# ZHANGKEON/DIS-YOLO

Hardware: AMD Instinct MI355X
Metric: train images/sec @576x576 bf16 (higher is better)
Workload: dtype bf16

## Files before the change

dis-yolo_amd/csrc/conv_common.h:

```cpp
#pragma once
#include <utility>
#include "common.h"

namespace dyconv {
struct ConvParams {
  const bf16* x0;
  const bf16* x1;
  const bf16* w;
  const float* scale;
  const float* shift;
  const bf16* residual;
  void* y;
  float* stats;
  const bf16* bn_x;
  const float* bn_scale;
  const float* bn_shift;
  const float* bn_mean;
  const float* bn_rstd;
  float* bn_part;
  float bn_alpha;
  int B, H, W, C0, C1, Cin;
  int Ho, Wo, Cout;
  int ks, stride, pad_t, pad_l, dmask, dshift;
  int M, K, nk;
// ... 7 lines not shown
  float alpha;
  void* y_act;
  const float* gamma;
  const float* beta;
  float* mm;
  float* mv;
  float* o_scale;
  float* o_shift;
  float* o_mean;
  float* o_rstd;
  float* dgamma;
  float* dbeta;
  unsigned* csync;
  float bn_decay, bn_eps;
  double inv_count;
};

template <int BK>
static __device__ __forceinline__ int swz(int row, int chunk) {
  if (BK == 32) return chunk ^ ((0x78 >> (((row >> 2) & 3) * 2)) & 3);
  return chunk ^ ((row >> 1) & 7);
}

static __device__ __forceinline__ int swz_any(int row, int chunk) { return chunk ^ (((row >> 2) & 1) << 1); }

typedef int i32x4 __attribute__((ext_vector_type(4)));
constexpr unsigned OOB = 0x80000000u;
template <int LDS_IMM>
static __device__ __forceinline__ void dma16(unsigned voff, i32x4 srd, unsigned soff, unsigned lds_base) {
  asm volatile("s_mov_b32 m0, %3\n\ts_nop 0\n\tbuffer_load_dwordx4 %0, %1, %2 offen lds"
// ... 183 lines not shown
```

dis-yolo_amd/csrc/conv_igemm.hip:

```cpp
#include <utility>
#include "common.h"
#include "conv_common.h"
#include "runtime.h"

using namespace dyconv;

namespace {

template <int BM, int BN, int WM, int WN, int BK, int ST, int KS, int KG = 1, int EPI = 0>
__global__ __launch_bounds__(WM* WN * 64 * KG, (BM == 128 && BN == 128) ? 3 : 1) void conv_igemm_kernel(ConvParams p) {
#ifdef HALO_PROBE
  long long gp_t[5];
  gp_t[0] = (long long)__builtin_amdgcn_s_memtime();
  gp_t[4] = (long long)__builtin_amdgcn_s_memrealtime();
#endif
  constexpr int NW = WM * WN;
  constexpr int T = NW * 64;
  constexpr int WTM = BM / WM, WTN = BN / WN;
  constexpr int MI = WTM / 16, NI = WTN / 16;
  constexpr int ROWB = BK * 2;
  constexpr int CPR = ROWB / 16;
  constexpr int SLAB = 1024 * NW;
  constexpr int A_BYTES = (BM * ROWB + SLAB - 1) / SLAB * SLAB;
  constexpr int B_BYTES = (BN * ROWB + SLAB - 1) / SLAB * SLAB;
// ... 1439 lines not shown
        const int idx = r_ * 64 + lane;
        const int r16 = idx / CPR8, ch = idx % CPR8;
        const int m = __shfl(m_of[t], r16, 64);
        const int n = n0 + ch * 8;
        const uint4 o = *reinterpret_cast<const uint4*>(sw + (t * 16 + r16) * ROWP + ch * 16);
        unsigned off = (m >= 0 && n < p.Cout) ? (unsigned)(((size_t)m * p.Cout + n) * 2) : OOB;
#ifdef DY_PROBE
        if (p.flags & 0x80000) off = OOB;
#endif
        buffer_store16(o, off, srdy);
      }
    }
  }
}

template <int NI>
__global__ __launch_bounds__(512) void conv1x1_stream_kernel(ConvParams p, int ngroups) {
  constexpr int NW = 8, U = 2;
  constexpr int BN = NI * 16;
  constexpr int ROWP = BN * 2 + 16;
  constexpr int STG = U * 16 * ROWP;
  constexpr int MAXKS = 6;
  extern __shared__ __attribute__((aligned(16))) char smem[];
  const int tid = threadIdx.x;
  const int lane = tid & 63;
  const int wave = __builtin_amdgcn_readfirstlane(tid >> 6);
  const int frow = lane & 15, cq = lane >> 4;
  const int K = p.K, ks32 = K >> 5;
  const int wpitch = K * 2 + 16;
  char* const wl = smem;
  char* const stg = smem + ((BN * wpitch + 15) & ~15);
  for (int c = tid; c < BN * (K >> 3); c += NW * 64) {
    const int n = c / (K >> 3), kc = c - n * (K >> 3);
    uint4 v = uint4{0, 0, 0, 0};
    if (n < p.Cout) v = *reinterpret_cast<const uint4*>(p.w + (size_t)n * K + kc * 8);
    *reinterpret_cast<uint4*>(wl + n * wpitch + kc * 16) = v;
  }
  float esc[NI][4], esh[NI][4];
#pragma unroll
  for (int j = 0; j < NI; ++j)
#pragma unroll
    for (int r = 0; r < 4; ++r) {
      const int n = j * 16 + cq * 4 + r;
      esc[j][r] = (p.scale && n < p.Cout) ? p.scale[n] : 1.f;
      esh[j][r] = (p.shift && n < p.Cout) ? p.shift[n] : 0.f;
    }
  __syncthreads();
  const bool f32out = p.flags & DISYOLO_CONV_OUT_F32;
  const bool do_stats = p.flags & DISYOLO_CONV_STATS;
  const bool vec_ok = (p.Cout & 7) == 0;
  const bool use_res = p.residual != nullptr;
  const int H1 = p.H >> 1, W1 = p.W >> 1;
  const int ks0 = p.C0 >> 5;
  float s1[NI][4], s2[NI][4];
#pragma unroll
  for (int j = 0; j < NI; ++j)
#pragma unroll
    for (int r = 0; r < 4; ++r) s1[j][r] = s2[j][r] = 0.f;
  char* const sw = stg + wave * STG;

  for (int g = blockIdx.x * NW + wave; g < ngroups; g += gridDim.x * NW) {
    int m_of[U];
    bf16x8 xf[U][MAXKS];
#pragma unroll
// ... 10 lines not shown
        a1 = p.x1 + ((size_t)(b * H1 + (y >> 1)) * W1 + (x >> 1)) * p.C1 + cq * 8;
      }
#pragma unroll
      for (int k = 0; k < MAXKS; ++k)
        if (k < ks32) xf[u][k] = *reinterpret_cast<const bf16x8*>(k < ks0 ? a0 + k * 32 : a1 + (k - ks0) * 32);
    }
    uint2 rres[U][NI];
    if (use_res) {
#pragma unroll
      for (int u = 0; u < U; ++u)
#pragma unroll
        for (int j = 0; j < NI; ++j) {
          const int n = j * 16 + cq * 4;
          rres[u][j] = *reinterpret_cast<const uint2*>(p.residual + (size_t)(m_of[u] >= 0 ? m_of[u] : 0) * p.Cout + (n + 3 < p.Cout ? n : 0));
        }
    }
    f32x4 acc[U][NI];
#pragma unroll
    for (int u = 0; u < U; ++u)
#pragma unroll
      for (int j = 0; j < NI; ++j) acc[u][j] = f32x4{0.f, 0.f, 0.f, 0.f};
#pragma unroll
    for (int k = 0; k < MAXKS; ++k) {
      if (k < ks32) {
        bf16x8 wf[NI];
#pragma unroll
        for (int j = 0; j < NI; ++j) wf[j] = *reinterpret_cast<const bf16x8*>(wl + (j * 16 + frow) * wpitch + (k * 4 + cq) * 16);
#pragma unroll
        for (int u = 0; u < U; ++u)
#pragma unroll
// ... 37 lines not shown
            for (int r = 0; r < 4; ++r)
              if (n + r < p.Cout) {
                float o = v[r];
                if (use_res && !(n + 3 < p.Cout)) o += (float)p.residual[off + r];
                if (f32out)
                  reinterpret_cast<float*>(p.y)[off + r] = o;
                else
                  reinterpret_cast<bf16*>(p.y)[off + r] = (bf16)o;
              }
          }
        } else {
          uint2 o2;
          o2.x = pack2(v[0], v[1]);
          o2.y = pack2(v[2], v[3]);
          *reinterpret_cast<uint2*>(sw + (u * 16 + frow) * ROWP + n * 2) = o2;
        }
      }
    if (!(f32out || !vec_ok)) {
      __builtin_amdgcn_fence(__ATOMIC_RELEASE, "wavefront");
      __builtin_amdgcn_wave_barrier();
      __builtin_amdgcn_fence(__ATOMIC_ACQUIRE, "wavefront");
      constexpr int CPR8 = BN / 8;
      constexpr int RPF = (U * 16 * CPR8 + 63) / 64;
      const int cpr = p.Cout >> 3;
      bf16* yo = reinterpret_cast<bf16*>(p.y);
#pragma unroll
      for (int r_ = 0; r_ < RPF; ++r_) {
        const int idx = r_ * 64 + lane;
        const int row = idx / CPR8, ch = idx % CPR8;
        const int m = g * (U * 16) + row;
        if (idx < U * 16 * CPR8 && ch < cpr && m < p.M)
          *reinterpret_cast<uint4*>(yo + (size_t)m * p.Cout + ch * 8) = *reinterpret_cast<const uint4*>(sw + row * ROWP + ch * 16);
      }
      __builtin_amdgcn_fence(__ATOMIC_RELEASE, "wavefront");
      __builtin_amdgcn_wave_barrier();
      __builtin_amdgcn_fence(__ATOMIC_ACQUIRE, "wavefront");
    }
  }
  if (do_stats) {
    float* red = reinterpret_cast<float*>(stg + NW * STG);
#pragma unroll
    for (int j = 0; j < NI; ++j)
#pragma unroll
      for (int r = 0; r < 4; ++r) {
        float a = s1[j][r], b2 = s2[j][r];
#pragma unroll
        for (int o = 1; o < 16; o <<= 1) {
          a += __shfl_xor(a, o, 64);
          b2 += __shfl_xor(b2, o, 64);
        }
        if (frow == 0) {
          const int nl = j * 16 + cq * 4 + r;
          red[(wave * BN + nl) * 2 + 0] = a;
          red[(wave * BN + nl) * 2 + 1] = b2;
        }
      }
    __syncthreads();
    for (int nl = tid; nl < BN; nl += NW * 64) {
      if (nl < p.Cout) {
        float a = 0.f, b2 = 0.f;
#pragma unroll
        for (int w_ = 0; w_ < NW; ++w_) {
          a += red[(w_ * BN + nl) * 2 + 0];
          b2 += red[(w_ * BN + nl) * 2 + 1];
        }
        stats_out(p, blockIdx.x, nl, a, b2);
      }
    }
  }
}

struct Patch {
  int ph, pw;
};
Patch pick_patch(int H, int W, int max_frags, int max_halo) {
  Patch best{0, 0};
  int best_area = 0, best_halo = 1 << 30;
  for (int ph = 1; ph <= H; ++ph) {
    if (H % ph) continue;
    for (int pw = 1; pw <= W; ++pw) {
      if (W % pw) continue;
// ... 53 lines not shown
    if (hipGetDevice(&dev) == hipSuccess) (void)hipDeviceGetAttribute(&n, hipDeviceAttributeMultiprocessorCount, dev);
    return n > 0 ? n : 256;
  }();
  int G = ncu / q.tilesN;
  if (G < 1) G = 1;
  if (G > q.tilesM) G = q.tilesM;
  hipLaunchKernelGGL((conv_stream_kernel<NW, FW, NI>), dim3(G * q.tilesN), dim3(NW * 64), lds, s, q, pt.ph, pt.pw, tilesY,
                     tilesX, G);
  DY_CHECK_LAUNCH();
  return DISYOLO_OK;
}

bool stream1x1_ok(const disyolo_conv_desc* d) {
  if (d->ksize != 1 || d->stride != 1 || d->in_div != 1 || d->Ho != d->H || d->Wo != d->W) return false;
  if (d->Cout > 64 || d->C0 % 32 || d->C1 % 32 || d->C0 + d->C1 > 192) return false;
  if (d->flags & DISYOLO_CONV_BN_BWD_STATS) return false;
  return true;
}
int stream1x1_blocks(int M) {
  const int groups = ceil_div(M, 32);
  int blocks = ceil_div(groups, 8 * 4);
  if (blocks > 512) blocks = 512;
  if (blocks < 1) blocks = 1;
  return blocks;
}
template <int NI>
int launch_stream1x1_n(const ConvParams& p, hipStream_t s) {
  constexpr int BN = NI * 16;
  const size_t wbytes = ((size_t)BN * (p.K * 2 + 16) + 15) & ~(size_t)15;
  const size_t lds = wbytes + (size_t)8 * 2 * 16 * (BN * 2 + 16) + (size_t)8 * BN * 8;
  static bool attr_set = false;
  if (!attr_set) {
    (void)hipFuncSetAttribute(reinterpret_cast<const void*>(&conv1x1_stream_kernel<NI>), hipFuncAttributeMaxDynamicSharedMemorySize,
                              (int)(64 * (192 * 2 + 16) + 8 * 2 * 16 * (64 * 2 + 16) + 8 * 64 * 8));
    attr_set = true;
  }
  hipLaunchKernelGGL((conv1x1_stream_kernel<NI>), dim3(stream1x1_blocks(p.M)), dim3(512), lds, s, p, ceil_div(p.M, 32));
  DY_CHECK_LAUNCH();
  return DISYOLO_OK;
}
int launch_stream1x1(const ConvParams& p, hipStream_t s) {
  if (p.Cout <= 16) return launch_stream1x1_n<1>(p, s);
  if (p.Cout <= 32) return launch_stream1x1_n<2>(p, s);
  return launch_stream1x1_n<4>(p, s);
}

struct LaunchQuery {
  bool active = false, have = false, want_bwd = false, want_fused = false;
  int grid = 0, rows = 0, bn = 0, resident = 0;
};
thread_local LaunchQuery tl_query;
template <class K>
int resident_blocks(K kernel, int threads, size_t lds) {
  int dev = 0, cus = 0, occ = 0;
  if (hipGetDevice(&dev) != hipSuccess) return 0;
  if (hipDeviceGetAttribute(&cus, hipDeviceAttributeMultiprocessorCount, dev) != hipSuccess) return 0;
  if (hipOccupancyMaxActiveBlocksPerMultiprocessor(&occ, reinterpret_cast<const void*>(kernel), threads, lds) != hipSuccess) {
    (void)hipGetLastError();
    return 0;
// ... 248 lines not shown
      if (halo_ok(d, id, pt)) return sel;
    } else {
      return sel;
    }
    sel = pick_auto(d, M);
  }
  return sel;
}

extern "C" int disyolo_conv2d_bn_bwd_stats_ok(const disyolo_conv_desc* d) {
  if (!d || (d->flags & DISYOLO_CONV_OUT_F32) || d->Cout % 8) return 0;
  if (conv_c16_shape(d)) return 0;
  const int sel = resolve_sel(d, d->B * d->Ho * d->Wo, nullptr);
  int id = sel & 0xff;
  if ((id >= 16 && id < 20) || id == 24 || id == 25) return 1;
  if (!is_gemm_tile(id) || d->in_div != 1) return 0;
  {
    const char* e = getenv("DISYOLO_BN_BWD_STATS_GEMM");
    if (!(e && e[0] == '1')) return 0;
  }
  const bool bk64 = (d->C0 % 64 == 0) && (d->C1 % 64 == 0) && !(sel & 0x100);
  id = resolve_tile(id, bk64, d->ksize * d->ksize * (d->C0 + d->C1));
  if (id == 12) return 1;
  return d->ksize == 1 && (id == 1 || id == 2 || id == 3 || id == 6 || id == 9 || id == 10 || id == 11) ? 1 : 0;
}

extern "C" int disyolo_conv2d_stats_rows(const disyolo_conv_desc* d) {
  if (!d) return DISYOLO_E_ARG;
  const int M = d->B * d->Ho * d->Wo;
  if (conv_c16_shape(d)) return conv_c16_stats_rows(d);
  Patch pt;
  const int id = resolve_sel(d, M, &pt) & 0xff;
  if (id == 24 || id == 25) {
    FlatGeom g;
    return flat_ok(d, id, &g) ? g.tilesM : DISYOLO_E_ARG;
  }
  if (id == 21) return stream1x1_blocks(M);
  if (!is_gemm_tile(id)) return d->B * (d->H / pt.ph) * (d->W / pt.pw);
  const int bm = tile_bm(id);
// ... 94 lines not shown

extern "C" int disyolo_dgrad_s2_quad_ok(int B, int Hdy, int Wdy, int Cdy, int C) {
  return (B > 0 && Hdy > 0 && Wdy > 0 && Cdy % 64 == 0 && C % 8 == 0 && (4 * C) % 128 == 0 && C <= 64 &&
          (int64_t)B * Hdy * Wdy * 4 * C * 2 < (1LL << 31) && (int64_t)B * Hdy * Wdy * Cdy * 2 < (1LL << 31)) ? 1 : 0;
}

extern "C" int disyolo_dgrad_s2_quad(const void* dy, const void* wq, void* dx, const void* residual, int B, int Hdy, int Wdy,
                                     int Cdy, int C, void* stream) {
  DY_REQUIRE(dy && wq && dx, "dgrad_s2_quad: null pointer");
  DY_REQUIRE(disyolo_dgrad_s2_quad_ok(B, Hdy, Wdy, Cdy, C) == 1, "dgrad_s2_quad: needs Cdy %% 64 == 0, C in {32, 64}");
  DY_RECORD_OR_RUN([=](void* s) { return disyolo_dgrad_s2_quad(dy, wq, dx, residual, B, Hdy, Wdy, Cdy, C, s); });
  ConvParams p;
  p.x0 = (const bf16*)dy; p.x1 = nullptr; p.w = (const bf16*)wq;
  p.scale = nullptr; p.shift = nullptr; p.residual = (const bf16*)residual; p.y = dx; p.stats = nullptr;
  p.bn_x = nullptr; p.bn_scale = p.bn_shift = p.bn_mean = p.bn_rstd = nullptr; p.bn_part = nullptr; p.bn_alpha = 0.f;
  p.B = B; p.H = Hdy; p.W = Wdy; p.C0 = Cdy; p.C1 = 0; p.Cin = Cdy;
  p.Ho = Hdy; p.Wo = Wdy; p.Cout = 4 * C;
  p.ks = 3; p.stride = 1; p.pad_t = 1; p.pad_l = 1; p.dmask = 0; p.dshift = 0;
  p.M = B * Hdy * Wdy;
  p.K = 9 * Cdy;
  p.bytes0 = (unsigned)((size_t)B * Hdy * Wdy * Cdy * 2);
  p.bytes1 = 0;
  p.bytesw = (unsigned)((size_t)4 * C * 9 * Cdy * 2);
  p.nk = 0;
  p.flags = 0;
  p.alpha = 0.f;
  p.tilesM = p.tilesN = 0;
  p.xcd_n = 0; p.halo_split = 0;
  p.pcls = 0; p.Mc = 0; p.tilesMc = 0;
  p.tapmask = 0x1b;
// ... 71 lines not shown
  p.residual = (const bf16*)d->residual;
  p.y = d->y;
  p.stats = d->stats;
  p.bn_x = nullptr; p.bn_scale = p.bn_shift = p.bn_mean = p.bn_rstd = nullptr; p.bn_part = nullptr; p.bn_alpha = 0.f;
  if (d->flags & DISYOLO_CONV_BN_BWD_STATS) {
    DY_REQUIRE(d->bn_x && d->bn_scale && d->bn_shift && d->bn_mean && d->bn_rstd && d->bn_partials,
               "conv: BN_BWD_STATS flag with a null bn_* pointer");
    DY_REQUIRE((d->flags & DISYOLO_CONV_BN_BWD_FUSED) || disyolo_conv2d_bn_bwd_stats_ok(d) == 1,
               "conv: BN_BWD_STATS needs a patch kernel (tile 16-19, 24, 25 on a shape it covers) or a GEMM tile with that epilogue "
               "(ask disyolo_conv2d_bn_bwd_stats_ok), bf16 output, Cout %% 8 == 0");
    DY_REQUIRE(!(d->flags & DISYOLO_CONV_BN_BWD_FUSED) || (!(d->flags & (DISYOLO_CONV_OUT_F32 | DISYOLO_CONV_STATS | DISYOLO_CONV_LEAKY)) &&
                                                          !d->scale && !d->shift && d->Cout % 8 == 0),
               "conv: BN_BWD_FUSED needs a plain bf16 data-gradient conv (no scale / shift / LEAKY / STATS), Cout %% 8 == 0");
    p.bn_x = (const bf16*)d->bn_x; p.bn_scale = d->bn_scale; p.bn_shift = d->bn_shift; p.bn_mean = d->bn_mean;
    p.bn_rstd = d->bn_rstd; p.bn_part = d->bn_partials; p.bn_alpha = d->bn_alpha;
  }
  p.B = d->B; p.H = d->H; p.W = d->W; p.C0 = d->C0; p.C1 = d->C1; p.Cin = d->C0 + d->C1;
  p.Ho = d->Ho; p.Wo = d->Wo; p.Cout = d->Cout;
  p.ks = d->ksize; p.stride = d->stride; p.pad_t = d->pad_t; p.pad_l = d->pad_l;
  p.dmask = d->in_div - 1; p.dshift = d->in_div == 2 ? 1 : 0;
  p.M = d->B * d->Ho * d->Wo;
  p.K = d->ksize * d->ksize * p.Cin;
  p.bytes0 = (unsigned)((size_t)d->B * d->H * d->W * d->C0 * 2);
  p.bytes1 = (unsigned)((size_t)d->B * (d->H / 2) * (d->W / 2) * d->C1 * 2);
  p.bytesw = (unsigned)((size_t)d->Cout * p.K * 2);
  p.nk = 0;
  p.flags = d->flags;
  p.alpha = d->alpha;
  p.tilesM = p.tilesN = 0;
  p.xcd_n = 0; p.halo_split = 0;
// ... 34 lines not shown
```

dis-yolo_amd/lib.py:

```python
from __future__ import annotations

import ctypes as C
import os
from typing import Optional

import numpy as np
import torch

_HERE = os.path.dirname(os.path.abspath(__file__))
LIB_PATH = os.environ.get("DISYOLO_LIB", os.path.join(_HERE, "libdisyolo_hip.so"))

GRAD_LD = 32
ROI_MAX = 16
ROI_W = 12
K_MAPS = (3, 5, 7)
MASK_STRIDES = (1, 2, 4)


def roi_w(k: int) -> int:
    return 2 * (k + 1) + 4


def block32_post(k: int) -> int:
    return {3: 1, 5: 2, 7: 3}[k]
CONV_LEAKY, CONV_OUT_F32, CONV_STATS, CONV_BN_BWD_STATS, CONV_BN_FUSED, CONV_BN_BWD_FUSED = 1, 2, 4, 8, 16, 32


class DisyoloError(RuntimeError):
    pass


class ConvDesc(C.Structure):
    _fields_ = [
        ("B", C.c_int32), ("H", C.c_int32), ("W", C.c_int32),
        ("C0", C.c_int32), ("C1", C.c_int32),
        ("Ho", C.c_int32), ("Wo", C.c_int32), ("Cout", C.c_int32),
        ("ksize", C.c_int32), ("stride", C.c_int32),
        ("pad_t", C.c_int32), ("pad_l", C.c_int32),
        ("in_div", C.c_int32), ("flags", C.c_int32),
        ("alpha", C.c_float), ("tile", C.c_int32),
# ... 7 lines not shown
        ("bn_moving_mean", C.c_void_p), ("bn_moving_var", C.c_void_p),
        ("bn_out_scale", C.c_void_p), ("bn_out_shift", C.c_void_p), ("bn_out_mean", C.c_void_p), ("bn_out_rstd", C.c_void_p),
        ("bn_dgamma", C.c_void_p), ("bn_dbeta", C.c_void_p), ("cluster_sync", C.c_void_p),
    ]


_SIGS = {
    "disyolo_version": (C.c_int, []),
    "disyolo_last_error": (C.c_char_p, []),
    "disyolo_conv_desc_size": (C.c_size_t, []),
    "disyolo_find_contours": (C.c_int, [C.c_void_p, C.c_int, C.c_int, C.c_void_p, C.c_int64, C.c_void_p, C.c_void_p, C.c_int,
                                        C.POINTER(C.c_int), C.POINTER(C.c_int64)]),
    "disyolo_conv2d_stats_rows": (C.c_int, [C.POINTER(ConvDesc)]),
    "disyolo_conv2d_bn_bwd_stats_ok": (C.c_int, [C.POINTER(ConvDesc)]),
    "disyolo_conv2d_bn_fused_ok": (C.c_int, [C.POINTER(ConvDesc)]),
    "disyolo_cluster_sync_words": (C.c_int, [C.c_int]),
    "disyolo_cluster_sync_error": (C.c_int, [C.c_void_p, C.c_int]),
    "disyolo_conv2d_fwd": (C.c_int, [C.POINTER(ConvDesc), C.c_void_p]),
    "disyolo_conv2d_tile": (C.c_int, [C.POINTER(ConvDesc)] + [C.POINTER(C.c_int)] * 4),
    "disyolo_conv_first_fwd": (C.c_int, [C.c_void_p] * 5 + [C.c_int] * 4 + [C.c_float, C.c_void_p]),
    "disyolo_conv12_fused_ok": (C.c_int, [C.c_int] * 3),
    "disyolo_conv12_fused_fwd": (C.c_int, [C.c_void_p] * 8 + [C.c_int] * 3 + [C.c_float, C.c_void_p]),
    "disyolo_block32_fused_ok": (C.c_int, [C.c_int] * 6),
    "disyolo_block64_fused_ok": (C.c_int, [C.c_int] * 4),
    "disyolo_pack_quad": (C.c_int, [C.c_void_p, C.c_void_p, C.c_int, C.c_int, C.c_void_p]),
    "disyolo_dgrad_s2_quad_ok": (C.c_int, [C.c_int] * 5),
    "disyolo_dgrad_s2_quad": (C.c_int, [C.c_void_p] * 4 + [C.c_int] * 5 + [C.c_void_p]),
    "disyolo_block64_fused_fwd": (C.c_int, [C.c_void_p] * 8 + [C.c_int] * 4 + [C.c_float, C.c_void_p]),
    "disyolo_block32_fused_fwd": (C.c_int, [C.c_void_p, C.c_void_p, C.c_int, C.c_int] + [C.c_void_p] * 6 + [C.c_int] +
                                  [C.c_void_p] * 3 + [C.c_int] * 3 + [C.c_float, C.c_void_p]),
# ... 228 lines not shown
        if lane == 1:
            return self.side_stream(device)
        if lane not in self._lanes:
            self._lanes[lane] = torch.cuda.ExternalStream(load().disyolo_cmdlist_lane_stream(self.h, lane), device=device)
        return self._lanes[lane]


def same_pads(size: int, k: int, s: int):
    out = -(-size // s)
    total = max((out - 1) * s + k - size, 0)
    return out, total // 2


def make_conv_desc(x0, w_packed, y, ksize, stride, *, x1=None, scale=None, shift=None, residual=None, stats=None,
                   leaky=False, out_f32=False, alpha=0.1, tile=0, in_div=1, pads=None, out_hw=None,
                   bn_bwd=None, bn_fused=None, bn_bwd_fused=None) -> ConvDesc:
    B, H, W, C0 = x0.shape
    C1 = 0 if x1 is None else x1.shape[3]
    if out_hw is None:
        Ho, pt = same_pads(H, ksize, stride)
        Wo, pl = same_pads(W, ksize, stride)
    else:
        Ho, Wo = out_hw
        pt, pl = pads
    if pads is not None:
        pt, pl = pads
    d = ConvDesc()
    d.B, d.H, d.W, d.C0, d.C1 = B, H, W, C0, C1
    d.Ho, d.Wo, d.Cout = Ho, Wo, y.shape[-1]
    d.ksize, d.stride, d.pad_t, d.pad_l, d.in_div = ksize, stride, pt, pl, in_div
    d.flags = (CONV_LEAKY if leaky else 0) | (CONV_OUT_F32 if out_f32 else 0) | (CONV_STATS if stats is not None else 0)
# ... 11 lines not shown
        f = bn_fused
        if stats is None or leaky or scale is not None or shift is not None or residual is not None:
            raise DisyoloError("make_conv_desc(bn_fused=...): needs stats, and no scale / shift / leaky / residual")
        d.flags |= CONV_BN_FUSED
        d.y_act, d.bn_gamma, d.bn_beta = _p(f["y_act"]), _p(f["gamma"]), _p(f["beta"])
        d.bn_moving_mean, d.bn_moving_var = _p(f.get("mm")), _p(f.get("mv"))
        d.bn_out_scale, d.bn_out_shift, d.bn_out_mean, d.bn_out_rstd = _p(f["scale"]), _p(f["shift"]), _p(f["mean"]), _p(f["rstd"])
        d.bn_decay, d.bn_eps = f["decay"], f["eps"]
        d.cluster_sync = _p(f["sync"])
    if bn_bwd_fused is not None:
        f = bn_bwd_fused
        if bn_bwd is None:
            raise DisyoloError("make_conv_desc(bn_bwd_fused=...): needs bn_bwd")
        d.flags |= CONV_BN_BWD_FUSED
        d.bn_dgamma, d.bn_dbeta, d.cluster_sync = _p(f["dgamma"]), _p(f["dbeta"]), _p(f["sync"])
    d._keepalive = (x0, x1, w_packed, scale, shift, residual, y, stats, bn_bwd, bn_fused, bn_bwd_fused)
    return d


def conv2d_bn_fused_ok(d: ConvDesc) -> bool:
    return load().disyolo_conv2d_bn_fused_ok(C.byref(d)) == 1


def cluster_sync_buffer(cout: int, device) -> torch.Tensor:
    return torch.zeros(load().disyolo_cluster_sync_words(cout), dtype=torch.int32, device=device)


def cluster_sync_error(buf: torch.Tensor, cout: int) -> int:
    return load().disyolo_cluster_sync_error(_p(buf), cout)


def conv2d_bn_bwd_stats_ok(d: ConvDesc) -> bool:
    return load().disyolo_conv2d_bn_bwd_stats_ok(C.byref(d)) == 1


def conv2d_stats_rows(d: ConvDesc) -> int:
    r = load().disyolo_conv2d_stats_rows(C.byref(d))
    if r < 0:
        raise DisyoloError("conv2d_stats_rows: bad descriptor")
    return r


def conv_shape_key(d: ConvDesc):
    return (d.B, d.H, d.W, d.C0, d.C1, d.Ho, d.Wo, d.Cout, d.ksize, d.stride, d.in_div)
# ... 110 lines not shown
        raise DisyoloError("conv2d_tile: bad descriptor")
    return tid, bm.value, bn.value, bk.value, st.value


def conv2d_fwd(d: ConvDesc) -> None:
    if TUNER is not None:
        TUNER.launch(d)
        return
    if TIMER is not None:
        if not hasattr(d, "_tname"):
            tid, bm, bn, bk, st = conv2d_tile(d)
            if tid in (24, 25):
                d._tname = "conv_flat_kernel<%s,2,%d>" % ("2,3,2,1" if tid == 24 else "4,3,1,2", st)
            elif tid == 21:
                d._tname = "conv1x1_stream_kernel<%d>" % (bn // 16)
            elif tid == 20:
                d._tname = "conv_stream_kernel<8,3,4>"
            elif tid >= 16:
                d._tname = "conv_halo_kernel<%d,3,%d>" % (4 if tid == 17 else 8, 2 if tid == 18 else 1 if tid == 19 else 4)
            else:
                d._tname = "conv_igemm_kernel<%d,%d,%d,%d,%d,%d,%d,%d,%d>" % ((bm, bn) + _WAVES.get(tid, (0, 0)) +
                                                                               (bk, st, d.ksize, 2 if 13 <= tid <= 15 else 1,
                                                                                1 if d.flags & CONV_BN_BWD_FUSED else 0))
        TIMER.run(d._tname, conv_flops(d), lambda: _check(load().disyolo_conv2d_fwd(C.byref(d), _stream()),
                                                           "conv2d_fwd"), conv_bytes(d))
        return
    _check(load().disyolo_conv2d_fwd(C.byref(d), _stream()), "conv2d_fwd")


def conv2d_fp8_fwd(d: ConvDesc, w8, escale, eshift, y8, out_scale: float, y16=None, residual8=None,
# ... 594 lines not shown
```

dis-yolo_amd/net.py:

```python
from __future__ import annotations

from typing import Dict, List, Optional, Sequence, Tuple

import math
import json
import contextlib
import os
import sys
import numpy as np
import torch

from . import config as cfg
from . import lib as L

BF16 = torch.bfloat16
F32 = torch.float32

WGRAD_GROUP = 3
OPT_CHUNK_ELEMS = 8_000_000
PIPE_LANE = 2


class Layer:
    __slots__ = ("idx", "cin", "cout", "k", "stride", "kind", "src", "src_up", "shortcut", "lock", "H", "W", "Ho",
                 "Wo", "w", "bias", "gamma", "beta", "mm", "mv", "scale", "shift", "mean", "rstd", "wp", "wdg", "raw",
                 "act", "stats", "stats_rows", "desc", "grad", "grad_set", "need_grad", "dw", "dbias", "dgamma",
                 "dbeta", "dx", "pad_t", "pad_l", "dgrad_descs", "wgrad_desc", "cout_pad",
                 "act8", "w8", "s_w", "s_out", "escale", "desc8", "dual16", "bn_sums", "bwd_local", "bwd_global", "bwd_part", "bwd_part_rows", "wq",
                 "csync", "fused_fwd", "csync_bwd", "fused_bwd")

    def __init__(self, idx, cin, cout, k, stride, kind, src, src_up=None, shortcut=None):
        self.idx, self.cin, self.cout, self.k, self.stride, self.kind = idx, cin, cout, k, stride, kind
        self.src, self.src_up, self.shortcut = src, src_up, shortcut
        for s in self.__slots__[9:]:
            setattr(self, s, None)


MASK_STRIDES = (4, 2, 1)


def build_topology(num_class: int, k_map: int, mask_stride: int = 2) -> List[Layer]:
    if mask_stride not in MASK_STRIDES:
        raise ValueError("mask_stride must be one of %s (got %r)" % (", ".join(map(str, MASK_STRIDES)), mask_stride))
    out_depth = (num_class + 5) * 3
# ... 127 lines not shown
        self.sync_bn = False
        self._rec = None
        self._prog = None
        self._prog_marks = []
        self._graph = None
        self.opt_chunks = None
        self._overlap = False
        self._overlap_rec = False
        self._tail_open = False
        self._progs = None
        self.fuse_first_two = True
        self.fuse_blocks = True
        self.use_side_lane = os.environ.get("DISYOLO_SIDE_LANE", "1") != "0"
        self.bn_inkernel = os.environ.get("DISYOLO_BN_INKERNEL", "1") != "0"
        self.bn_inkernel_bwd = os.environ.get("DISYOLO_BN_INKERNEL_BWD", "0") == "1"
        self.bn_fuse_check = None
        self.tail_on_main = 0
        self.pair = bool(backbone_pair)
        self._half = 0
        self._pair_P = 0
        self._init_params(seed, xavier_locked)
        if self.pair:
            if not self.training or self.dtype != "bf16" or self.plan_only:
                raise L.DisyoloError("backbone_pair needs a bf16 training net")
            self._pair_P = self._backbone_prefix()
            if self._pair_P < 2:
                raise L.DisyoloError("backbone_pair needs a locked layer prefix (stage 1)")
        if not self.plan_only:
            self._plan(self.batchsize, self.image_size)

# ... 308 lines not shown
                        if l.stats.shape[0] < rows:
                            l.stats = torch.zeros(rows, l.cout, 2, dtype=F32, device=dev)
                        if l.csync is None:
                            l.csync = L.cluster_sync_buffer(l.cout, dev)
                        l.desc = L.make_conv_desc(x0, l.wp, l.raw, l.k, l.stride, x1=x1, stats=l.stats, tile=tile,
                                                  bn_fused=dict(y_act=l.act, gamma=l.gamma, beta=l.beta, mm=l.mm, mv=l.mv,
                                                                scale=l.scale, shift=l.shift, mean=l.mean, rstd=l.rstd,
                                                                decay=cfg.BN_DECAY, eps=cfg.BN_EPSILON, sync=l.csync),
                                                  alpha=cfg.ALPHA)
                        l.fused_fwd = True
            else:
                l.desc = L.make_conv_desc(x0, l.wp, l.act, l.k, l.stride, x1=x1, scale=l.scale, shift=l.shift,
                                          residual=res, leaky=True, alpha=cfg.ALPHA)
            if self.training and not l.lock:
                l.wgrad_desc = L.make_conv_desc(x0, l.wp, l.act, l.k, l.stride, x1=x1)

    FUSED_TILES_1x1 = (3, 2, 6, 10, 1, 12, 0x20c)
    FUSED_TILES_3x3 = (16, 18, 19, 12, 0x20c)

    def _fused_tile(self, make_desc, k: int, bwd: bool = False):
        best, best_blocks = None, -1
        for i, t in enumerate((0,) + (self.FUSED_TILES_3x3 if k == 3 else self.FUSED_TILES_1x1)):
            d = make_desc(t)
            tid, bm, bn, _, _ = L.conv2d_tile(d)
            if t and tid != (t & 0xff):
                continue
            if bwd:
                d.flags |= L.CONV_BN_BWD_FUSED
            ok = L.conv2d_bn_fused_ok(d)
            d.flags &= ~L.CONV_BN_BWD_FUSED
# ... 296 lines not shown
            return
        train_bn = is_training and self.training and (not l.lock) and l.kind != "lin"
        M = B * l.Ho * l.Wo
        res = self._input_of(l, l.shortcut) if l.shortcut is not None else None
        if l.idx == 1:
            if train_bn:
                L.conv_first_fwd(self.images, l.w, self._ones32, self._zeros32, l.raw, alpha=1.0)
                L.colstats(l.raw, l.stats, M, l.cout)
                self._bn_finalize(l, M)
                L.bn_act_fwd(l.raw, l.scale, l.shift, None, l.act, M, l.cout, cfg.ALPHA)
            else:
                if not l.lock and self.training:
                    L.bn_fold(l.gamma, l.beta, l.mm, l.mv, cfg.BN_EPSILON, l.scale, l.shift)
                L.conv_first_fwd(self.images, l.w, l.scale, l.shift, l.act, alpha=cfg.ALPHA)
            return
        if l.kind == "lin":
            L.conv2d_fwd(l.desc)
        elif train_bn:
            L.conv2d_fwd(l.desc)
            if l.fused_fwd and L.TUNER is None:
                return
            self._bn_finalize(l, M)
            L.bn_act_fwd(l.raw, l.scale, l.shift, res, l.act, M, l.cout, cfg.ALPHA)
        else:
            if self.training and not l.lock:
                L.bn_fold(l.gamma, l.beta, l.mm, l.mv, cfg.BN_EPSILON, l.scale, l.shift)
                d = L.make_conv_desc(self._input_of(l, l.src), l.wp, l.act, l.k, l.stride,
                                     x1=self._input_of(l, l.src_up) if l.src_up is not None else None,
                                     scale=l.scale, shift=l.shift, residual=res, leaky=True, alpha=cfg.ALPHA)
                L.conv2d_fwd(d)
            else:
                L.conv2d_fwd(l.desc)

    def _bn_finalize(self, l, M: int) -> None:
        rows = l.stats_rows
        if L.TUNER is not None:
            rows = L.TUNER.stats_rows.get(l.stats.data_ptr(), rows)
# ... 231 lines not shown
        first = not tgt.grad_set
        if "quad" in desc_kw and L.TUNER is None:
            ql = desc_kw["quad"]
            L.pack_quad(ql.w, ql.wq)
            L.dgrad_s2_quad(dx, ql.wq, tgt.grad, accumulate=not first)
            return
        res = None if (first or "tmp" in desc_kw) else tgt.grad
        d = L.make_conv_desc(dx, desc_kw["w"], out, k, 1, in_div=in_div, pads=desc_kw["pads"], out_hw=desc_kw["out_hw"],
                             residual=res)
        whole, tile_f = False, None
        if (final and L.TUNER is None and self.bn_inkernel and self.bn_inkernel_bwd and not self.sync_bn
                and self.bn_fuse_check is None and not self._shortcut_feeds_grad(tgt) and in_div == 1):
            tile_f = self._fused_tile(lambda t: L.make_conv_desc(dx, desc_kw["w"], out, k, 1, in_div=in_div, pads=desc_kw["pads"],
                                                                 out_hw=desc_kw["out_hw"], residual=res, tile=t), k, bwd=True)
            whole = tile_f is not None
        if final and L.TUNER is None and not whole and L.conv2d_bn_bwd_stats_ok(d):
            rows = L.conv2d_stats_rows(d)
            need = rows * tgt.cout * 2
            if tgt.bwd_part is None or tgt.bwd_part.numel() < need:
                tgt.bwd_part = torch.empty(need, dtype=torch.float32, device=self.device)
            tgt.bwd_part_rows = rows
            d = L.make_conv_desc(dx, desc_kw["w"], out, k, 1, in_div=in_div, pads=desc_kw["pads"], out_hw=desc_kw["out_hw"],
                                 residual=res,
                                 bn_bwd=(tgt.raw, tgt.scale, tgt.shift, tgt.mean, tgt.rstd, tgt.bwd_part, cfg.ALPHA))
        elif whole:
            d = L.make_conv_desc(dx, desc_kw["w"], out, k, 1, in_div=in_div, pads=desc_kw["pads"], out_hw=desc_kw["out_hw"],
                                 residual=res, tile=tile_f)
            rows = L.conv2d_stats_rows(d)
            need = rows * tgt.cout * 2
            if tgt.bwd_part is None or tgt.bwd_part.numel() < need:
                tgt.bwd_part = torch.empty(need, dtype=torch.float32, device=self.device)
            if tgt.csync_bwd is None:
                tgt.csync_bwd = L.cluster_sync_buffer(tgt.cout, self.device)
            d = L.make_conv_desc(dx, desc_kw["w"], tgt.dx, k, 1, in_div=in_div, pads=desc_kw["pads"], out_hw=desc_kw["out_hw"],
                                 residual=res, tile=tile_f,
                                 bn_bwd=(tgt.raw, tgt.scale, tgt.shift, tgt.mean, tgt.rstd, tgt.bwd_part, cfg.ALPHA),
                                 bn_bwd_fused=dict(dgamma=tgt.dgamma, dbeta=tgt.dbeta, sync=tgt.csync_bwd))
            tgt.fused_bwd = True
# ... 557 lines not shown
```

include/disyolo.h:

```cpp
#ifndef DISYOLO_H
#define DISYOLO_H

#include <stddef.h>
#include <stdint.h>

#ifdef __cplusplus
extern "C" {
#endif

#define DISYOLO_OK 0
#define DISYOLO_E_ARG (-1)
#define DISYOLO_E_WORKSPACE (-2)
#define DISYOLO_E_HIP (-3)

#define DISYOLO_GRAD_LD 32
#define DISYOLO_ROI_MAX 16
#define DISYOLO_ROI_W 12
#define DISYOLO_ROI_W_K(k) (2 * ((k) + 1) + 4)

int disyolo_version(void);
const char* disyolo_last_error(void);

enum {
  DISYOLO_CONV_LEAKY = 1,
  DISYOLO_CONV_OUT_F32 = 2,
  DISYOLO_CONV_STATS = 4,
  DISYOLO_CONV_BN_BWD_STATS = 8,
  DISYOLO_CONV_BN_FUSED = 16,
  DISYOLO_CONV_BN_BWD_FUSED = 32,
};

typedef struct disyolo_conv_desc {
  int32_t B, H, W;
  int32_t C0, C1;
  int32_t Ho, Wo, Cout;
  int32_t ksize, stride;
  int32_t pad_t, pad_l;
  int32_t in_div;
  int32_t flags;
  float alpha;
  int32_t tile;
  const void* x0;
  const void* x1;
  const void* w;
// ... 17 lines not shown
  float* bn_moving_var;
  float* bn_out_scale;
  float* bn_out_shift;
  float* bn_out_mean;
  float* bn_out_rstd;
  float* bn_dgamma;
  float* bn_dbeta;
  uint32_t* cluster_sync;
} disyolo_conv_desc;

int disyolo_find_contours(const uint8_t* binary, int h, int w, int32_t* points_xy, int64_t max_points,
                          int32_t* contour_start, int32_t* hierarchy, int max_contours, int* n_contours,
                          int64_t* n_points);
size_t disyolo_conv_desc_size(void);
int disyolo_conv2d_bn_bwd_stats_ok(const disyolo_conv_desc* d);
int disyolo_conv2d_bn_fused_ok(const disyolo_conv_desc* d);
int disyolo_cluster_sync_words(int Cout);
int disyolo_cluster_sync_error(const uint32_t* cluster_sync, int Cout);
int disyolo_conv2d_stats_rows(const disyolo_conv_desc* d);
int disyolo_conv2d_fwd(const disyolo_conv_desc* d, void* stream);
int disyolo_conv2d_tile(const disyolo_conv_desc* d, int* bm, int* bn, int* bk, int* stages);

int disyolo_conv_first_fwd(const float* images, const float* w_hwio, const float* scale,
                           const float* shift, void* y_bf16, int B, int H, int W, int Cout,
                           float alpha, void* stream);

int disyolo_conv12_fused_ok(int B, int H, int W);
int disyolo_conv12_fused_fwd(const float* images, const float* w1_hwio, const float* scale1, const float* shift1,
                             const void* w2_packed, const float* scale2, const float* shift2, void* y_bf16, int B, int H,
                             int W, float alpha, void* stream);
// ... 222 lines not shown
```

Baseline: 2160.

## Fold producer BN+leaky into streaming 1x1 conv prologue and add BN-bwd stats variant

Adds a BN_IN mode to the streaming 1x1 conv kernel. The consumer conv reads the producer's raw pre-BN output, applies the folded scale/shift and leaky activation in registers, writes the activated tensor for later readers, and feeds it straight to the GEMM. This skips the separate bn_act_fwd kernel for eligible layers, removing one full read and write pass over the activation. A BNB variant that accumulates BN-backward partial sums inside the same kernel is also added, but it stays off by default behind an environment flag. The cost is a larger LDS footprint, more kernel instantiations, and extra global stores from the conv prologue.

```diff
diff --git a/dis-yolo_amd/csrc/conv_common.h b/dis-yolo_amd/csrc/conv_common.h
--- a/dis-yolo_amd/csrc/conv_common.h
+++ b/dis-yolo_amd/csrc/conv_common.h
@@ -45,6 +45,10 @@
   unsigned* csync;
   float bn_decay, bn_eps;
   double inv_count;
+  const float* in_scale;
+  const float* in_shift;
+  bf16* act_out;
+  float in_alpha;
 };
 
 template <int BK>
diff --git a/dis-yolo_amd/csrc/conv_igemm.hip b/dis-yolo_amd/csrc/conv_igemm.hip
--- a/dis-yolo_amd/csrc/conv_igemm.hip
+++ b/dis-yolo_amd/csrc/conv_igemm.hip
@@ -1477,13 +1477,14 @@
   }
 }
 
-template <int NI>
+template <int NI, bool BNIN = false, bool BNB = false>
 __global__ __launch_bounds__(512) void conv1x1_stream_kernel(ConvParams p, int ngroups) {
   constexpr int NW = 8, U = 2;
   constexpr int BN = NI * 16;
   constexpr int ROWP = BN * 2 + 16;
   constexpr int STG = U * 16 * ROWP;
-  constexpr int MAXKS = 6;
+  constexpr int MAXKS = BNB ? 2 : 6;
+  static_assert(!(BNIN && BNB), "one folded batch-norm pass per instance");
   extern __shared__ __attribute__((aligned(16))) char smem[];
   const int tid = threadIdx.x;
   const int lane = tid & 63;
@@ -1508,9 +1509,25 @@
       esc[j][r] = (p.scale && n < p.Cout) ? p.scale[n] : 1.f;
       esh[j][r] = (p.shift && n < p.Cout) ? p.shift[n] : 0.f;
     }
+  float* const bnc = reinterpret_cast<float*>(stg + NW * STG + NW * BN * 8);
+  if constexpr (BNIN) {
+    for (int c = tid; c < K; c += NW * 64) {
+      bnc[c] = p.in_scale[c];
+      bnc[K + c] = p.in_shift[c];
+    }
+  }
+  if constexpr (BNB) {
+    for (int c = tid; c < BN; c += NW * 64) {
+      const bool ok = c < p.Cout;
+      bnc[c] = ok ? p.bn_scale[c] : 0.f;
+      bnc[BN + c] = ok ? p.bn_shift[c] : 0.f;
+      bnc[2 * BN + c] = ok ? p.bn_mean[c] : 0.f;
+      bnc[3 * BN + c] = ok ? p.bn_rstd[c] : 0.f;
+    }
+  }
   __syncthreads();
-  const bool f32out = p.flags & DISYOLO_CONV_OUT_F32;
-  const bool do_stats = p.flags & DISYOLO_CONV_STATS;
+  const bool f32out = !BNB && (p.flags & DISYOLO_CONV_OUT_F32);
+  const bool do_stats = !BNB && (p.flags & DISYOLO_CONV_STATS);
   const bool vec_ok = (p.Cout & 7) == 0;
   const bool use_res = p.residual != nullptr;
   const int H1 = p.H >> 1, W1 = p.W >> 1;
@@ -1551,6 +1568,38 @@
           const int n = j * 16 + cq * 4;
           rres[u][j] = *reinterpret_cast<const uint2*>(p.residual + (size_t)(m_of[u] >= 0 ? m_of[u] : 0) * p.Cout + (n + 3 < p.Cout ? n : 0));
         }
+    }
+    uint2 bx[U][BNB ? NI : 1];
+    if constexpr (BNB) {
+#pragma unroll
+      for (int u = 0; u < U; ++u)
+#pragma unroll
+        for (int j = 0; j < NI; ++j) {
+          const int n = j * 16 + cq * 4;
+          bx[u][j] = (m_of[u] >= 0 && n < p.Cout) ? *reinterpret_cast<const uint2*>(p.bn_x + (size_t)m_of[u] * p.Cout + n) : uint2{0, 0};
+        }
+    }
+    if constexpr (BNIN) {
+#pragma unroll
+      for (int k = 0; k < MAXKS; ++k) {
+        if (k < ks32) {
+          const int c0 = k * 32 + cq * 8;
+          const float4 a0 = *reinterpret_cast<const float4*>(bnc + c0), a1 = *reinterpret_cast<const float4*>(bnc + c0 + 4);
+          const float4 h0 = *reinterpret_cast<const float4*>(bnc + K + c0), h1 = *reinterpret_cast<const float4*>(bnc + K + c0 + 4);
+          const float sc[8] = {a0.x, a0.y, a0.z, a0.w, a1.x, a1.y, a1.z, a1.w};
+          const float sh[8] = {h0.x, h0.y, h0.z, h0.w, h1.x, h1.y, h1.z, h1.w};
+#pragma unroll
+          for (int u = 0; u < U; ++u) {
+            float v[8];
+            unpack8(__builtin_bit_cast(uint4, xf[u][k]), v);
+#pragma unroll
+            for (int i = 0; i < 8; ++i) v[i] = leaky(v[i] * sc[i] + sh[i], p.in_alpha);
+            const uint4 o = pack8(v);
+            if (m_of[u] >= 0) *reinterpret_cast<uint4*>(p.act_out + (size_t)m_of[u] * p.C0 + c0) = o;
+            xf[u][k] = __builtin_bit_cast(bf16x8, o);
+          }
+        }
+      }
     }
     f32x4 acc[U][NI];
 #pragma unroll
@@ -1618,6 +1667,26 @@
           o2.x = pack2(v[0], v[1]);
           o2.y = pack2(v[2], v[3]);
           *reinterpret_cast<uint2*>(sw + (u * 16 + frow) * ROWP + n * 2) = o2;
+          if constexpr (BNB) {
+            const bool live = m_of[u] >= 0 && n < p.Cout;
+            const float4 sc4 = *reinterpret_cast<const float4*>(bnc + n), sh4 = *reinterpret_cast<const float4*>(bnc + BN + n);
+            const float4 mu4 = *reinterpret_cast<const float4*>(bnc + 2 * BN + n), rs4 = *reinterpret_cast<const float4*>(bnc + 3 * BN + n);
+            const float bsc[4] = {sc4.x, sc4.y, sc4.z, sc4.w}, bsh[4] = {sh4.x, sh4.y, sh4.z, sh4.w};
+            const float bmu[4] = {mu4.x, mu4.y, mu4.z, mu4.w}, brs[4] = {rs4.x, rs4.y, rs4.z, rs4.w};
+            const uint2 xx = bx[u][j];
+            const float va[4] = {__builtin_bit_cast(float, o2.x << 16), __builtin_bit_cast(float, o2.x & 0xffff0000u),
+                                 __builtin_bit_cast(float, o2.y << 16), __builtin_bit_cast(float, o2.y & 0xffff0000u)};
+            const float vx[4] = {__builtin_bit_cast(float, xx.x << 16), __builtin_bit_cast(float, xx.x & 0xffff0000u),
+                                 __builtin_bit_cast(float, xx.y << 16), __builtin_bit_cast(float, xx.y & 0xffff0000u)};
+#pragma unroll
+            for (int r = 0; r < 4; ++r) {
+              const float z = vx[r] * bsc[r] + bsh[r];
+              const float g = (live ? va[r] : 0.f) * (z > 0.f ? 1.f : p.bn_alpha);
+              const float xh = (vx[r] - bmu[r]) * brs[r];
+              s1[j][r] += g;
+              s2[j][r] += g * xh;
+            }
+          }
         }
       }
     if (!(f32out || !vec_ok)) {
@@ -1641,7 +1710,7 @@
       __builtin_amdgcn_fence(__ATOMIC_ACQUIRE, "wavefront");
     }
   }
-  if (do_stats) {
+  if (do_stats || BNB) {
     float* red = reinterpret_cast<float*>(stg + NW * STG);
 #pragma unroll
     for (int j = 0; j < NI; ++j)
@@ -1668,7 +1737,10 @@
           a += red[(w_ * BN + nl) * 2 + 0];
           b2 += red[(w_ * BN + nl) * 2 + 1];
         }
-        stats_out(p, blockIdx.x, nl, a, b2);
+        if constexpr (BNB)
+          bnpart_out(p, blockIdx.x, nl, a, b2);
+        else
+          stats_out(p, blockIdx.x, nl, a, b2);
       }
     }
   }
@@ -1752,7 +1824,10 @@
 bool stream1x1_ok(const disyolo_conv_desc* d) {
   if (d->ksize != 1 || d->stride != 1 || d->in_div != 1 || d->Ho != d->H || d->Wo != d->W) return false;
   if (d->Cout > 64 || d->C0 % 32 || d->C1 % 32 || d->C0 + d->C1 > 192) return false;
-  if (d->flags & DISYOLO_CONV_BN_BWD_STATS) return false;
+  if (d->flags & DISYOLO_CONV_BN_BWD_STATS) {
+    if (d->C1 != 0 || d->C0 > 64 || d->Cout % 8) return false;
+    if ((d->flags & (DISYOLO_CONV_OUT_F32 | DISYOLO_CONV_STATS | DISYOLO_CONV_LEAKY | DISYOLO_CONV_BN_IN)) || d->scale || d->shift) return false;
+  }
   return true;
 }
 int stream1x1_blocks(int M) {
@@ -1762,25 +1837,31 @@
   if (blocks < 1) blocks = 1;
   return blocks;
 }
-template <int NI>
+template <int NI, bool BNIN = false, bool BNB = false>
 int launch_stream1x1_n(const ConvParams& p, hipStream_t s) {
   constexpr int BN = NI * 16;
   const size_t wbytes = ((size_t)BN * (p.K * 2 + 16) + 15) & ~(size_t)15;
-  const size_t lds = wbytes + (size_t)8 * 2 * 16 * (BN * 2 + 16) + (size_t)8 * BN * 8;
+  const size_t lds = wbytes + (size_t)8 * 2 * 16 * (BN * 2 + 16) + (size_t)8 * BN * 8 + (BNIN ? (size_t)p.K * 8 : 0) + (BNB ? (size_t)BN * 16 : 0);
   static bool attr_set = false;
   if (!attr_set) {
-    (void)hipFuncSetAttribute(reinterpret_cast<const void*>(&conv1x1_stream_kernel<NI>), hipFuncAttributeMaxDynamicSharedMemorySize,
-                              (int)(64 * (192 * 2 + 16) + 8 * 2 * 16 * (64 * 2 + 16) + 8 * 64 * 8));
+    (void)hipFuncSetAttribute(reinterpret_cast<const void*>(&conv1x1_stream_kernel<NI, BNIN, BNB>), hipFuncAttributeMaxDynamicSharedMemorySize,
+                              (int)(64 * (192 * 2 + 16) + 8 * 2 * 16 * (64 * 2 + 16) + 8 * 64 * 8 + 192 * 8));
     attr_set = true;
   }
-  hipLaunchKernelGGL((conv1x1_stream_kernel<NI>), dim3(stream1x1_blocks(p.M)), dim3(512), lds, s, p, ceil_div(p.M, 32));
+  hipLaunchKernelGGL((conv1x1_stream_kernel<NI, BNIN, BNB>), dim3(stream1x1_blocks(p.M)), dim3(512), lds, s, p, ceil_div(p.M, 32));
   DY_CHECK_LAUNCH();
   return DISYOLO_OK;
 }
+template <bool BNIN, bool BNB>
+int launch_stream1x1_f(const ConvParams& p, hipStream_t s) {
+  if (p.Cout <= 16) return launch_stream1x1_n<1, BNIN, BNB>(p, s);
+  if (p.Cout <= 32) return launch_stream1x1_n<2, BNIN, BNB>(p, s);
+  return launch_stream1x1_n<4, BNIN, BNB>(p, s);
+}
 int launch_stream1x1(const ConvParams& p, hipStream_t s) {
-  if (p.Cout <= 16) return launch_stream1x1_n<1>(p, s);
-  if (p.Cout <= 32) return launch_stream1x1_n<2>(p, s);
-  return launch_stream1x1_n<4>(p, s);
+  if (p.flags & DISYOLO_CONV_BN_IN) return launch_stream1x1_f<true, false>(p, s);
+  if (p.flags & DISYOLO_CONV_BN_BWD_STATS) return launch_stream1x1_f<false, true>(p, s);
+  return launch_stream1x1_f<false, false>(p, s);
 }
 
 struct LaunchQuery {
@@ -2059,6 +2140,11 @@
   const int sel = resolve_sel(d, d->B * d->Ho * d->Wo, nullptr);
   int id = sel & 0xff;
   if ((id >= 16 && id < 20) || id == 24 || id == 25) return 1;
+  if (id == 21) {
+    disyolo_conv_desc c = *d;
+    c.flags |= DISYOLO_CONV_BN_BWD_STATS;
+    return stream1x1_ok(&c) ? 1 : 0;
+  }
   if (!is_gemm_tile(id) || d->in_div != 1) return 0;
   {
     const char* e = getenv("DISYOLO_BN_BWD_STATS_GEMM");
@@ -2068,6 +2154,12 @@
   id = resolve_tile(id, bk64, d->ksize * d->ksize * (d->C0 + d->C1));
   if (id == 12) return 1;
   return d->ksize == 1 && (id == 1 || id == 2 || id == 3 || id == 6 || id == 9 || id == 10 || id == 11) ? 1 : 0;
+}
+
+extern "C" int disyolo_conv2d_bn_in_ok(const disyolo_conv_desc* d) {
+  if (!d || d->C1 != 0 || conv_c16_shape(d)) return 0;
+  if (d->flags & (DISYOLO_CONV_BN_BWD_STATS | DISYOLO_CONV_BN_FUSED | DISYOLO_CONV_BN_BWD_FUSED)) return 0;
+  return (resolve_sel(d, d->B * d->Ho * d->Wo, nullptr) & 0xff) == 21 ? 1 : 0;
 }
 
 extern "C" int disyolo_conv2d_stats_rows(const disyolo_conv_desc* d) {
@@ -2192,6 +2284,7 @@
   p.x0 = (const bf16*)dy; p.x1 = nullptr; p.w = (const bf16*)wq;
   p.scale = nullptr; p.shift = nullptr; p.residual = (const bf16*)residual; p.y = dx; p.stats = nullptr;
   p.bn_x = nullptr; p.bn_scale = p.bn_shift = p.bn_mean = p.bn_rstd = nullptr; p.bn_part = nullptr; p.bn_alpha = 0.f;
+  p.in_scale = p.in_shift = nullptr; p.act_out = nullptr; p.in_alpha = 0.f;
   p.B = B; p.H = Hdy; p.W = Wdy; p.C0 = Cdy; p.C1 = 0; p.Cin = Cdy;
   p.Ho = Hdy; p.Wo = Wdy; p.Cout = 4 * C;
   p.ks = 3; p.stride = 1; p.pad_t = 1; p.pad_l = 1; p.dmask = 0; p.dshift = 0;
@@ -2293,6 +2386,13 @@
                "conv: BN_BWD_FUSED needs a plain bf16 data-gradient conv (no scale / shift / LEAKY / STATS), Cout %% 8 == 0");
     p.bn_x = (const bf16*)d->bn_x; p.bn_scale = d->bn_scale; p.bn_shift = d->bn_shift; p.bn_mean = d->bn_mean;
     p.bn_rstd = d->bn_rstd; p.bn_part = d->bn_partials; p.bn_alpha = d->bn_alpha;
+  }
+  p.in_scale = p.in_shift = nullptr; p.act_out = nullptr; p.in_alpha = 0.f;
+  if (d->flags & DISYOLO_CONV_BN_IN) {
+    DY_REQUIRE(d->bn_scale && d->bn_shift && d->y_act, "conv: BN_IN flag with a null bn_scale / bn_shift / y_act");
+    DY_REQUIRE(disyolo_conv2d_bn_in_ok(d) == 1,
+               "conv: BN_IN needs the streaming 1x1 kernel (tile 21) on a single-source conv (ask disyolo_conv2d_bn_in_ok)");
+    p.in_scale = d->bn_scale; p.in_shift = d->bn_shift; p.act_out = (bf16*)d->y_act; p.in_alpha = d->bn_alpha;
   }
   p.B = d->B; p.H = d->H; p.W = d->W; p.C0 = d->C0; p.C1 = d->C1; p.Cin = d->C0 + d->C1;
   p.Ho = d->Ho; p.Wo = d->Wo; p.Cout = d->Cout;
diff --git a/dis-yolo_amd/lib.py b/dis-yolo_amd/lib.py
--- a/dis-yolo_amd/lib.py
+++ b/dis-yolo_amd/lib.py
@@ -24,6 +24,7 @@
 def block32_post(k: int) -> int:
     return {3: 1, 5: 2, 7: 3}[k]
 CONV_LEAKY, CONV_OUT_F32, CONV_STATS, CONV_BN_BWD_STATS, CONV_BN_FUSED, CONV_BN_BWD_FUSED = 1, 2, 4, 8, 16, 32
+CONV_BN_IN = 64
 
 
 class DisyoloError(RuntimeError):
@@ -61,6 +62,7 @@
     "disyolo_conv2d_stats_rows": (C.c_int, [C.POINTER(ConvDesc)]),
     "disyolo_conv2d_bn_bwd_stats_ok": (C.c_int, [C.POINTER(ConvDesc)]),
     "disyolo_conv2d_bn_fused_ok": (C.c_int, [C.POINTER(ConvDesc)]),
+    "disyolo_conv2d_bn_in_ok": (C.c_int, [C.POINTER(ConvDesc)]),
     "disyolo_cluster_sync_words": (C.c_int, [C.c_int]),
     "disyolo_cluster_sync_error": (C.c_int, [C.c_void_p, C.c_int]),
     "disyolo_conv2d_fwd": (C.c_int, [C.POINTER(ConvDesc), C.c_void_p]),
@@ -319,7 +321,7 @@
 
 def make_conv_desc(x0, w_packed, y, ksize, stride, *, x1=None, scale=None, shift=None, residual=None, stats=None,
                    leaky=False, out_f32=False, alpha=0.1, tile=0, in_div=1, pads=None, out_hw=None,
-                   bn_bwd=None, bn_fused=None, bn_bwd_fused=None) -> ConvDesc:
+                   bn_bwd=None, bn_fused=None, bn_bwd_fused=None, bn_in=None) -> ConvDesc:
     B, H, W, C0 = x0.shape
     C1 = 0 if x1 is None else x1.shape[3]
     if out_hw is None:
@@ -361,7 +363,15 @@
             raise DisyoloError("make_conv_desc(bn_bwd_fused=...): needs bn_bwd")
         d.flags |= CONV_BN_BWD_FUSED
         d.bn_dgamma, d.bn_dbeta, d.cluster_sync = _p(f["dgamma"]), _p(f["dbeta"]), _p(f["sync"])
-    d._keepalive = (x0, x1, w_packed, scale, shift, residual, y, stats, bn_bwd, bn_fused, bn_bwd_fused)
+    if bn_in is not None:
+        if x1 is not None or tuple(bn_in[2].shape) != tuple(x0.shape):
+            raise DisyoloError("make_conv_desc(bn_in=...): single source, act_out shaped like x0")
+        d.flags |= CONV_BN_IN
+        if bn_bwd is not None or bn_fused is not None or bn_bwd_fused is not None:
+            raise DisyoloError("make_conv_desc(bn_in=...): not together with bn_bwd / bn_fused / bn_bwd_fused")
+        d.bn_scale, d.bn_shift, d.y_act = (_p(t) for t in bn_in[:3])
+        d.bn_alpha = bn_in[3]
+    d._keepalive = (x0, x1, w_packed, scale, shift, residual, y, stats, bn_bwd, bn_fused, bn_bwd_fused, bn_in)
     return d
 
 
@@ -375,6 +385,10 @@
 
 def cluster_sync_error(buf: torch.Tensor, cout: int) -> int:
     return load().disyolo_cluster_sync_error(_p(buf), cout)
+
+
+def conv2d_bn_in_ok(d: ConvDesc) -> bool:
+    return load().disyolo_conv2d_bn_in_ok(C.byref(d)) == 1
 
 
 def conv2d_bn_bwd_stats_ok(d: ConvDesc) -> bool:
@@ -515,6 +529,9 @@
                 d._tname = "conv_flat_kernel<%s,2,%d>" % ("2,3,2,1" if tid == 24 else "4,3,1,2", st)
             elif tid == 21:
                 d._tname = "conv1x1_stream_kernel<%d>" % (bn // 16)
+                if d.flags & (CONV_BN_IN | CONV_BN_BWD_STATS):
+                    d._tname = "conv1x1_stream_kernel<%d,%d,%d>" % (bn // 16, 1 if d.flags & CONV_BN_IN else 0,
+                                                                    1 if d.flags & CONV_BN_BWD_STATS else 0)
             elif tid == 20:
                 d._tname = "conv_stream_kernel<8,3,4>"
             elif tid >= 16:
diff --git a/dis-yolo_amd/net.py b/dis-yolo_amd/net.py
--- a/dis-yolo_amd/net.py
+++ b/dis-yolo_amd/net.py
@@ -27,7 +27,7 @@
                  "act", "stats", "stats_rows", "desc", "grad", "grad_set", "need_grad", "dw", "dbias", "dgamma",
                  "dbeta", "dx", "pad_t", "pad_l", "dgrad_descs", "wgrad_desc", "cout_pad",
                  "act8", "w8", "s_w", "s_out", "escale", "desc8", "dual16", "bn_sums", "bwd_local", "bwd_global", "bwd_part", "bwd_part_rows", "wq",
-                 "csync", "fused_fwd", "csync_bwd", "fused_bwd")
+                 "csync", "fused_fwd", "csync_bwd", "fused_bwd", "act_by", "desc_in")
 
     def __init__(self, idx, cin, cout, k, stride, kind, src, src_up=None, shortcut=None):
         self.idx, self.cin, self.cout, self.k, self.stride, self.kind = idx, cin, cout, k, stride, kind
@@ -185,6 +185,9 @@
         self.use_side_lane = os.environ.get("DISYOLO_SIDE_LANE", "1") != "0"
         self.bn_inkernel = os.environ.get("DISYOLO_BN_INKERNEL", "1") != "0"
         self.bn_inkernel_bwd = os.environ.get("DISYOLO_BN_INKERNEL_BWD", "0") == "1"
+        self.bn_bwd_partials = True
+        self.stream_bn_in = os.environ.get("DISYOLO_STREAM_BN_IN", "1") != "0"
+        self.stream_bn_bwd = os.environ.get("DISYOLO_STREAM_BN_BWD_STATS", "0") == "1"
         self.bn_fuse_check = None
         self.tail_on_main = 0
         self.pair = bool(backbone_pair)
@@ -523,6 +526,28 @@
                                           residual=res, leaky=True, alpha=cfg.ALPHA)
             if self.training and not l.lock:
                 l.wgrad_desc = L.make_conv_desc(x0, l.wp, l.act, l.k, l.stride, x1=x1)
+        self._plan_stream_bn_in()
+
+    def _plan_stream_bn_in(self) -> None:
+        for l in self.layers:
+            l.act_by, l.desc_in = None, None
+        if not (self.training and self.stream_bn_in) or getattr(self, "plan_only", False):
+            return
+        for l in self.layers:
+            P = self.by_idx.get(l.src)
+            if (P is None or P.idx == 1 or l.src_up is not None or l.shortcut is not None or l.lock or l.fused_fwd
+                    or l.k != 1 or P.lock or P.kind == "lin" or P.shortcut is not None or P.fused_fwd or P.raw is None
+                    or P.idx in self.HEAD_LAYERS or l.idx in self.HEAD_LAYERS):
+                continue
+            readers = [x.idx for x in self.layers if P.idx in (x.src, x.src_up, x.shortcut)]
+            if min(readers) != l.idx or not L.conv2d_bn_in_ok(l.desc):
+                continue
+            bn_in = (P.scale, P.shift, P.act, cfg.ALPHA)
+            if l.kind == "lin":
+                l.desc_in = L.make_conv_desc(P.raw, l.wp, l.act, l.k, l.stride, shift=l.bias, out_f32=True, bn_in=bn_in)
+            else:
+                l.desc_in = L.make_conv_desc(P.raw, l.wp, l.raw, l.k, l.stride, stats=l.stats, bn_in=bn_in)
+            P.act_by = l.idx
 
     FUSED_TILES_1x1 = (3, 2, 6, 10, 1, 12, 0x20c)
     FUSED_TILES_3x3 = (16, 18, 19, 12, 0x20c)
@@ -849,13 +874,16 @@
                     L.bn_fold(l.gamma, l.beta, l.mm, l.mv, cfg.BN_EPSILON, l.scale, l.shift)
                 L.conv_first_fwd(self.images, l.w, l.scale, l.shift, l.act, alpha=cfg.ALPHA)
             return
+        desc = l.desc_in if (l.desc_in is not None and is_training and self.training and L.TUNER is None) else l.desc
         if l.kind == "lin":
-            L.conv2d_fwd(l.desc)
+            L.conv2d_fwd(desc)
         elif train_bn:
-            L.conv2d_fwd(l.desc)
+            L.conv2d_fwd(desc)
             if l.fused_fwd and L.TUNER is None:
                 return
             self._bn_finalize(l, M)
+            if l.act_by is not None and L.TUNER is None:
+                return
             L.bn_act_fwd(l.raw, l.scale, l.shift, res, l.act, M, l.cout, cfg.ALPHA)
         else:
             if self.training and not l.lock:
@@ -1117,14 +1145,23 @@
             tile_f = self._fused_tile(lambda t: L.make_conv_desc(dx, desc_kw["w"], out, k, 1, in_div=in_div, pads=desc_kw["pads"],
                                                                  out_hw=desc_kw["out_hw"], residual=res, tile=t), k, bwd=True)
             whole = tile_f is not None
-        if final and L.TUNER is None and not whole and L.conv2d_bn_bwd_stats_ok(d):
+        tile_s = 0
+        sums = final and L.TUNER is None and not whole and self.bn_bwd_partials
+        if sums and k == 1 and not self.stream_bn_bwd and L.conv2d_tile(d)[0] == 21:
+            sums = False
+        if sums and self.stream_bn_bwd and k == 1 and in_div == 1 and not L.conv2d_bn_bwd_stats_ok(d):
+            d21 = L.make_conv_desc(dx, desc_kw["w"], out, k, 1, in_div=in_div, pads=desc_kw["pads"], out_hw=desc_kw["out_hw"],
+                                   residual=res, tile=21)
+            if L.conv2d_tile(d21)[0] == 21 and L.conv2d_bn_bwd_stats_ok(d21):
+                d, tile_s = d21, 21
+        if sums and L.conv2d_bn_bwd_stats_ok(d):
             rows = L.conv2d_stats_rows(d)
             need = rows * tgt.cout * 2
             if tgt.bwd_part is None or tgt.bwd_part.numel() < need:
                 tgt.bwd_part = torch.empty(need, dtype=torch.float32, device=self.device)
             tgt.bwd_part_rows = rows
             d = L.make_conv_desc(dx, desc_kw["w"], out, k, 1, in_div=in_div, pads=desc_kw["pads"], out_hw=desc_kw["out_hw"],
-                                 residual=res,
+                                 residual=res, tile=tile_s,
                                  bn_bwd=(tgt.raw, tgt.scale, tgt.shift, tgt.mean, tgt.rstd, tgt.bwd_part, cfg.ALPHA))
         elif whole:
             d = L.make_conv_desc(dx, desc_kw["w"], out, k, 1, in_div=in_div, pads=desc_kw["pads"], out_hw=desc_kw["out_hw"],
diff --git a/include/disyolo.h b/include/disyolo.h
--- a/include/disyolo.h
+++ b/include/disyolo.h
@@ -28,6 +28,7 @@
   DISYOLO_CONV_BN_BWD_STATS = 8,
   DISYOLO_CONV_BN_FUSED = 16,
   DISYOLO_CONV_BN_BWD_FUSED = 32,
+  DISYOLO_CONV_BN_IN = 64,
 };
 
 typedef struct disyolo_conv_desc {
@@ -75,6 +76,7 @@
                           int64_t* n_points);
 size_t disyolo_conv_desc_size(void);
 int disyolo_conv2d_bn_bwd_stats_ok(const disyolo_conv_desc* d);
+int disyolo_conv2d_bn_in_ok(const disyolo_conv_desc* d);
 int disyolo_conv2d_bn_fused_ok(const disyolo_conv_desc* d);
 int disyolo_cluster_sync_words(int Cout);
 int disyolo_cluster_sync_error(const uint32_t* cluster_sync, int Cout);
```

Result: no change. 2154 (-0.3%).
